# ljj7975/honk

Hardware: AMD Instinct MI355X
Metric: 1s-clips/sec (whole node) + top-1 acc, res15 12-label Speech Commands (higher is better)
Workload: dtype f16x2

## Files before the change

### honk_amd/csrc/res_bf16p.inc

```

#ifndef HONK_PAIR_PDM
#define HONK_PAIR_PDM 0
#endif
#ifndef HONK_PAIR_PKRELU
#define HONK_PAIR_PKRELU 1
#endif
#ifndef HONK_PAIR_MIX
#define HONK_PAIR_MIX 1
#endif

struct Block16PArgs {
  __bf16* R;
  const char* wA;
  const char* wB;
  unsigned chunk_bytes;
  int nclips, H, W;
  int d, lgd, sB;
  int lag;
  int NRA, NRB;
  int slotb;
  int ppr;
  float* chsum;
  int padb;
  int ringpad;
};

template <int NT, int SP>
struct G16P {
  static constexpr int P = 64;
  static constexpr int ZB = 256;
  static constexpr int PXB = 16 * ((G16W<NT, SP>::CB / 16 + 1) / 4 * 4 + 2);
};
static constexpr int g16p_pxb(int NT, int SP) { return 16 * ((32 * NT * SP / 16 + 1) / 4 * 4 + 2); }

static constexpr int g16p_lds_bytes() { return 160 * 1024; }
static constexpr int g16p_zb_tbl() { return 1024; }
static constexpr int g16p_tr() { return 32; }
static constexpr int g16p_teb() { return 32; }
static constexpr int g16p_lds_extra(bool tbl, int wps, int slotb) {
  return tbl ? g16p_zb_tbl() + 1024 + wps * g16p_tr() * g16p_teb() + slotb : 256 + 1024;
}
static constexpr int g16p_sink_off(int zb) { return ((zb > g16p_zb_tbl() ? zb : g16p_zb_tbl()) + 255) / 256 * 256; }
static constexpr int g16p_shared_bytes(int zb) { return g16p_sink_off(zb) + 1024; }
static constexpr int g16p_stream_bytes(int ns, int slotb) {
  return ((g16p_lds_bytes() - g16p_shared_bytes(slotb)) / ns) / 256 * 256;
}

template <int NT, int SP, int PPR, int PPW, int NS, bool LM, int FM, int SCA = 0, int SCB = 0, bool LIN = false>
__device__ __forceinline__ void block16p_body(const Block16PArgs& a) {
  using G = G16W<NT, SP, FM>;
  using Q = G16P<NT, SP>;
  constexpr int KSA = G::KSA, CB = G::CB, CP = G::CP, P = Q::P;
  constexpr int PD0 = ((FM == 2 || SCA > 0) && KSA % 7 == 0 && NS == 1) ? 6 : G::PD;
  constexpr int NOA = PD0 + 1;
  constexpr int PD = PD0 > 2 ? PD0 - HONK_PAIR_PDM : PD0;
  constexpr int PXB = Q::PXB;
  constexpr int MAXR = (2 * PPW + PPR - 1) / PPR;
  static_assert(KSA > PPW + 1, "DMA pieces ride on k-steps 1 .. PPW");
  __shared__ __attribute__((aligned(16))) char lds[g16p_lds_bytes()];

  const int tid = threadIdx.x;
  const int lane = tid & 63;
  const int wave = __builtin_amdgcn_readfirstlane(tid >> 6);
  constexpr int WPS = LM ? 2 : 4;
  const int stream = wave / WPS;
  const int role = LM ? 0 : ((wave >> 1) & 1) ^ ((HONK_PAIR_MIX && NS == 2) ? (stream & 1) : 0);
  const int widx = wave & 1;
  const int g = lane >> 4;
  const int i16 = lane & 15;

  const int GR = gridDim.x;
  const int bid = blockIdx.x;
  const int w0 = (int)(((long)bid * a.nclips) / GR);
  const int w1 = (int)(((long)(bid + 1) * a.nclips) / GR);
  if (w1 <= w0) return;
  const int per = (w1 - w0 + NS - 1) / NS;
  const int s0 = min(w0 + stream * per, w1);
  const int s1 = min(s0 + per, w1);
  int c0 = s0, c1 = s1;
  const int H = a.H, W = a.W, d = a.d, lgd = a.lgd;
  const int RB = W * CB;
  const unsigned clip_bytes = (unsigned)(H * RB);
  int rows_total = (c1 - c0) * H;
  int total = rows_total * W;
  const int qd = H >> lgd, rem = H & (d - 1);
  const int q1 = qd + 1;
  constexpr bool TBL = FM == 2 || (FM == 0 && SCA != 0);
  constexpr bool PADC = TBL && (LM || SCA > 0);
  const int padb = PADC ? a.padb : 0;
  constexpr int ZB = TBL ? g16p_zb_tbl() : Q::ZB;
  constexpr bool SHZ = NS > 1 && TBL && !LM;
  const int sbase = SHZ ? g16p_shared_bytes(a.slotb + a.ringpad) + stream * g16p_stream_bytes(NS, a.slotb + a.ringpad)
                        : stream * (g16p_lds_bytes() / NS);
  const int ringA = sbase, ringB = sbase + a.NRA * a.slotb;
  const int zoff = SHZ ? 0 : sbase + (a.NRA + a.NRB) * a.slotb + a.ringpad;
  const int dummy = SHZ ? g16p_sink_off(a.slotb + a.ringpad) : zoff + ZB;
  const int nsteps = ((LM ? 1 : per) * H * W + a.lag + P - 1) / P + 1;

  if ((wave & (WPS - 1)) == 0) {
    if constexpr (TBL) *(u32x4*)(lds + zoff + lane * 16) = u32x4{0u, 0u, 0u, 0u};
    else *(unsigned*)(lds + zoff + lane * 4) = 0u;
  }
  if constexpr (TBL) {
    const int zs = SHZ ? 0 : dummy + 1024 + WPS * g16p_tr() * g16p_teb();
    for (int o = ((wave & (WPS - 1)) * 64 + lane) * 16; o < a.slotb + a.ringpad; o += WPS * 1024)
      *(u32x4*)(lds + zs + o) = u32x4{0u, 0u, 0u, 0u};
    const int rings = PADC ? (a.NRA + a.NRB) * a.slotb + a.ringpad : 0;
    for (int o = ((wave & (WPS - 1)) * 64 + lane) * 16; o < rings; o += WPS * 1024)
      *(u32x4*)(lds + sbase + o) = u32x4{0u, 0u, 0u, 0u};
  }
  __builtin_amdgcn_s_waitcnt(0xc07f);
  __builtin_amdgcn_s_barrier();

  u32x4 wr[G::WP][KSA][NT];
  {
    const __amdgpu_buffer_rsrc_t wrs =
        __builtin_amdgcn_make_buffer_rsrc((void*)(role ? a.wB : a.wA), (short)0, G::WP * G::WPART, 0x00020000);
#pragma unroll
    for (int pt = 0; pt < G::WP; ++pt)
#pragma unroll
      for (int s = 0; s < KSA; ++s)
#pragma unroll
        for (int n = 0; n < NT; ++n) {
          const bool used = s < KSA - 1 || g < G::UGA;
          int voff = used ? lane * 16 : 0x40000000, soff = G::xfrag(pt, s, n);
          if (G::MERGE && s == KSA - 1 && pt == 0 && !used) {
            voff = (lane - 16 * G::UGA) * 16;
            soff = G::xfrag(1, s, n);
          }
          wr[pt][s][n] = __builtin_bit_cast(u32x4, __builtin_amdgcn_raw_buffer_load_b128(wrs, voff, soff, 0));
          if ((pt * KSA + s) * NT + n < (NS * WPS > 4 ? 32 : 64)) asm volatile("" : "+a"(wr[pt][s][n]));
        }
  }

  constexpr int CPT = 2 * NT;
  const int g16 = 16 * g;
  const int hi2 = g >= 2 ? -1 : 0;
  int lastc;
  {
    constexpr int S = KSA - 1, tA = (4 * S) / CPT;
    int cc[4];
#pragma unroll
    for (int gi = 0; gi < 4; ++gi) {
      const int gg = (G::MERGE && gi >= G::UGA) ? gi - G::UGA : gi;
      const int c = 4 * S + gg;
      cc[gi] = c < 18 * NT ? c - tA * CPT : 0;
    }
    const int ccg = g == 0 ? cc[0] : g == 1 ? cc[1] : g == 2 ? cc[2] : cc[3];
    lastc = 16 * ccg + 16 * CPT * tA - g16;
  }
  static_assert((4 * (KSA - 1) + 3) / CPT == (4 * (KSA - 1)) / CPT || 4 * (KSA - 1) + 3 >= 18 * NT,
                "the last k-step covers one tap");

  const int ring = role ? ringB : ringA;
  const int nr = role ? a.NRB : a.NRA;
  const int sr = role ? a.sB : 1;
  const int sc = role ? (a.sB << lgd) : d;
  const int scb = sc * PXB;

  struct Walk {
    int q, w, j, n, c;
    unsigned rowb;
    int sR, sO;
  };
  const unsigned dRB = (unsigned)(RB << lgd);
  const unsigned dclsd = (unsigned)RB - (unsigned)(qd - 1) * dRB, dcls1d = 0u - dRB;
  const unsigned dclip = clip_bytes - (unsigned)((d - 1) * RB) - (unsigned)(((d - 1) < rem ? q1 : qd) - 1) * dRB;
  const int ringRb = nr * a.slotb, ringOb = a.NRB * a.slotb, srb = sr * a.slotb;
  auto walk_init = [&](int q0) {
    Walk k;
    k.q = q0;
    const int qs = q0 >= 0 ? q0 : q0 + ((31 - q0) >> 5) * 32;
    const int r = qs / W;
    k.w = qs - r * W;
    const int cl = r / H;
    const int rl = r - cl * H;
    if (rl < rem * q1) {
      k.c = rl / q1;
      k.j = rl - k.c * q1;
      k.n = q1;
    } else {
      const int t = rl - rem * q1;
      const int cu = t / qd;
      k.c = rem + cu;
      k.j = t - cu * qd;
      k.n = qd;
    }
    k.rowb = (unsigned)(c0 + cl) * clip_bytes + (unsigned)((k.c + (k.j << lgd)) * RB);
    k.sR = (r % nr) * a.slotb;
    k.sO = (r % a.NRB) * a.slotb;
    return k;
  };
  auto row_adv = [&](Walk& k) {
    const int sR1 = k.sR + a.slotb, sO1 = k.sO + a.slotb;
    k.sR = sR1 == ringRb ? 0 : sR1;
    k.sO = sO1 == ringOb ? 0 : sO1;
    const int j1 = k.j + 1;
    const bool wj = j1 == k.n;
    const int c1 = k.c + (wj ? 1 : 0);
    const bool wc = c1 == d;
    unsigned inc = dRB;
    const unsigned dcls = dclsd + (k.n == q1 ? dcls1d : 0u);
    inc = wj ? dcls : inc;
    inc = wc ? dclip : inc;
    k.rowb += inc;
    k.j = wj ? 0 : j1;
    k.c = wc ? 0 : c1;
    k.n = k.c < rem ? q1 : qd;
  };
  constexpr bool WIDE = (PPR - 1) * 1024 >= 32 * PXB;
  auto walk_adv = [&](Walk& k) {
    if constexpr (WIDE) {
      const int w2 = k.w + (k.q >= 0 ? 32 : 0);
      const bool wrap = w2 >= W;
      k.w = wrap ? w2 - W : w2;
      const int sR1 = k.sR + (wrap ? a.slotb : 0), sO1 = k.sO + (wrap ? a.slotb : 0);
      k.sR = sR1 == ringRb ? 0 : sR1;
      k.sO = sO1 == ringOb ? 0 : sO1;
      const int j1 = k.j + (wrap ? 1 : 0);
      const bool wj = j1 == k.n;
      const int c1 = k.c + (wj ? 1 : 0);
      const bool wc = c1 == d;
      unsigned inc = wrap ? dRB : 0u;
      const unsigned dcls = dclsd + (k.n == q1 ? dcls1d : 0u);
      inc = wj ? dcls : inc;
      inc = wc ? dclip : inc;
      k.rowb += inc;
      k.j = wj ? 0 : j1;
      k.c = wc ? 0 : c1;
      k.n = k.c < rem ? q1 : qd;
    } else {
      if (k.q >= 0) {
        k.w += 32;
        while (k.w >= W) {
          k.w -= W;
          row_adv(k);
        }
      }
    }
    k.q += 32;
  };
  struct MG {
    int tq[9];
    unsigned pix;
    int lo;
  };
  auto geo = [&](const Walk& k) {
    MG m;
    const bool valid = k.q >= 0 && k.q < total;
    int sm = k.sR - srb, sp = k.sR + srb;
    sm = sm < 0 ? sm + ringRb : sm;
    sp = sp >= ringRb ? sp - ringRb : sp;
    const int wb = k.w * PXB + g16;
    const bool rok[3] = {valid && k.j >= sr, valid, valid && k.j + sr < k.n};
    const int rbase[3] = {ring + sm + wb, ring + k.sR + wb, ring + sp + wb};
    const bool cok[3] = {k.w >= sc, true, k.w + sc < W};
    const int zg = zoff + g16;
#pragma unroll
    for (int dy = 0; dy < 3; ++dy)
#pragma unroll
      for (int dx = 0; dx < 3; ++dx) {
        const int t = dy * 3 + dx;
        m.tq[t] = ((rok[dy] && cok[dx]) ? rbase[dy] + (dx - 1) * scb : zg) - 16 * CPT * t;
      }
    m.pix = valid ? k.rowb + (unsigned)(k.w * CB) : 0xF0000000u;
    m.lo = valid ? ringB + k.sO + k.w * PXB : dummy;
    return m;
  };

  constexpr int TR = g16p_tr(), TEB = g16p_teb();
  const int tbl = (SHZ ? sbase + (a.NRA + a.NRB) * a.slotb + a.ringpad : dummy + 1024) + (wave & (WPS - 1)) * (TR * TEB);
  const int zslot = SHZ ? 0 : dummy + 1024 + WPS * (TR * TEB);
  struct WalkT {
    int w, r;
    u32x4 e;
    int lo;
    int wb;
    bool okl, okr;
  };
  auto refill = [&](int tb) {
    const int r = tb + lane;
    int rb0 = zslot + padb, rb1 = zslot + padb, rb2 = zslot + padb, lo = -1;
    unsigned pix = 0xF0000000u;
    if (lane < TR && r >= 0 && r < rows_total) {
      const int cl = r / H, rl = r - cl * H;
      int c, j, n;
      if (rl < rem * q1) {
        c = rl / q1;
        j = rl - c * q1;
        n = q1;
      } else {
        const int t = rl - rem * q1, cu = t / qd;
        c = rem + cu;
        j = t - cu * qd;
        n = qd;
      }
      pix = (unsigned)(c0 + cl) * clip_bytes + (unsigned)((c + (j << lgd)) * RB);
      rb1 = ring + (r % nr) * a.slotb + padb;
      if (j >= sr) rb0 = ring + ((r - sr) % nr) * a.slotb + padb;
      if (j + sr < n) rb2 = ring + ((r + sr) % nr) * a.slotb + padb;
      lo = ringB + (r % a.NRB) * a.slotb + padb;
    }
    if (lane < TR) {
      char* e = lds + tbl + (r & (TR - 1)) * TEB;
      *(u32x4*)e = u32x4{(unsigned)rb0, (unsigned)rb1, (unsigned)rb2, pix};
      *(int*)(e + 16) = lo;
    }
  };
  auto floordiv = [](int x, int y) { return x >= 0 ? x / y : -((y - 1 - x) / y); };
  auto tread = [&](WalkT& k) {
    const char* e = lds + tbl + (k.r & (TR - 1)) * TEB;
    k.e = *(const u32x4*)e;
    k.lo = *(const int*)(e + 16);
    k.wb = __mul24(k.w, PXB) + g16;
    if constexpr (!PADC) {
      k.okl = k.w >= sc;
      k.okr = k.w + sc < W;
    }
  };
  auto walk_init_t = [&](int q0) {
    WalkT k;
    k.r = floordiv(q0, W);
    k.w = q0 - k.r * W;
    tread(k);
    return k;
  };
  constexpr int NWRAP = WIDE ? 1 : 3;
  auto walk_adv_t = [&](WalkT& k) {
    k.w += 32;
#pragma unroll
    for (int i = 0; i < NWRAP; ++i) {
      const bool wrap = k.w >= W;
      k.w = wrap ? k.w - W : k.w;
      k.r += wrap ? 1 : 0;
    }
    tread(k);
  };
  int tk[9];
#pragma unroll
  for (int t = 0; t < 9; ++t) tk[t] = (t % 3 - 1) * scb - 16 * CPT * t;
  const int zg0 = zoff + g16;
  auto scc_of = [](auto rolec) constexpr { return decltype(rolec)::value ? SCB : SCA; };
  auto biasc_of = [](auto rolec) constexpr {
    return (decltype(rolec)::value ? SCB : SCA) * PXB + 96;
  };
  auto geo_row = [&](auto rolec, const WalkT& k, MG& m, auto dyc) {
    constexpr int DY = decltype(dyc)::value;
    constexpr int SCC = scc_of(decltype(rolec){});
    const int rb = (int)k.e[DY] + k.wb;
    if constexpr (PADC && SCC > 0) {
      m.tq[DY] = rb - biasc_of(decltype(rolec){});
    } else if constexpr (PADC) {
#pragma unroll
      for (int dx = 0; dx < 3; ++dx) m.tq[DY * 3 + dx] = rb + tk[DY * 3 + dx];
    } else {
      const bool ok[3] = {k.okl, true, k.okr};
#pragma unroll
      for (int dx = 0; dx < 3; ++dx) m.tq[DY * 3 + dx] = ok[dx] ? rb + tk[DY * 3 + dx] : zg0;
    }
    if constexpr (DY == 2) {
      m.pix = k.e[3] + (unsigned)__mul24(k.w, CB);
      m.lo = k.lo >= 0 ? k.lo + k.wb - g16 : dummy;
    }
  };
  auto geo_t = [&](auto rolec, const WalkT& k) {
    MG m;
    static_for<3>([&](auto dyc) { geo_row(rolec, k, m, dyc); });
    return m;
  };
  auto lc_same = [&](auto rolec) { return hi2 & (scc_of(decltype(rolec){}) * PXB - 16 * CPT); };
  auto lc_next = [&](auto rolec) { return hi2 & (-2 * scc_of(decltype(rolec){}) * PXB - 16 * CPT); };
  auto aoff = [&](auto rolec, const int (&tq)[9], auto stc) {
    constexpr int S = decltype(stc)::value;
    constexpr int tA = (4 * S) / CPT;
    constexpr int SCC = scc_of(decltype(rolec){});
    if constexpr (PADC && SCC > 0) {
      if constexpr (S == KSA - 1) {
        return tq[tA / 3] + lastc - 16 * CPT * tA;
      } else {
        constexpr int tB = (4 * S + 3) / CPT;
        if constexpr (tA == tB) {
          return tq[tA / 3];
        } else if constexpr (tA / 3 == tB / 3) {
          return tq[tA / 3] + lc_same(rolec);
        } else {
          return ((tq[tB / 3] & hi2) | (tq[tA / 3] & ~hi2)) + lc_next(rolec);
        }
      }
    } else if constexpr (S == KSA - 1) {
      return tq[tA] + lastc - 64 * S;
    } else {
      constexpr int tB = (4 * S + 3) / CPT;
      if constexpr (tA == tB) {
        return tq[tA];
      } else {
        constexpr int GS = CPT * tB - 4 * S;
        static_assert(GS == 2, "NT = 3: every mixed k-step splits its lane groups 2 + 2");
        return (tq[tB] & hi2) | (tq[tA] & ~hi2);
      }
    }
  };

  auto imm_of = [](auto rolec, auto stc) constexpr {
    constexpr int S = decltype(stc)::value;
    constexpr int tA = (4 * S) / CPT;
    constexpr int SCC = decltype(rolec)::value ? SCB : SCA;
    constexpr int B = SCC * PXB + 96;
    if constexpr (S == KSA - 1) return B + (tA % 3 - 1) * SCC * PXB;
    else return B + (tA % 3 - 1) * SCC * PXB - 16 * CPT * tA + 64 * S;
  };

  u32x4 oa[NOA][SP];
  auto load_a = [&](auto rolec, const int (&tq)[9], auto stc, u32x4 (&o)[SP]) {
    constexpr int S = decltype(stc)::value;
    const int off = aoff(rolec, tq, stc);
    if constexpr (PADC && scc_of(decltype(rolec){}) > 0) {
      constexpr int IMM = imm_of(decltype(rolec){}, stc);
      static_assert(IMM >= 0 && IMM < 65536, "IMM: ds_read offset range");
#pragma unroll
      for (int pt = 0; pt < SP; ++pt) o[pt] = *(const u32x4*)(lds + off + IMM + pt * CP * 2);
    } else {
#pragma unroll
      for (int pt = 0; pt < SP; ++pt) o[pt] = *(const u32x4*)(lds + off + 64 * S + pt * CP * 2);
    }
  };

  f32x4 accs[2][NT];
  uint4 rvs[2][G::NRF][SP];
  unsigned ppix = 0xF0000000u;
  int plo = dummy;
#pragma unroll
  for (int q = 0; q < 2; ++q) {
#pragma unroll
    for (int n = 0; n < NT; ++n) accs[q][n] = f32x4{0.f, 0.f, 0.f, 0.f};
#pragma unroll
    for (int f = 0; f < G::NRF; ++f)
#pragma unroll
      for (int pt = 0; pt < SP; ++pt) rvs[q][f][pt] = uint4{0u, 0u, 0u, 0u};
  }
  const __amdgpu_buffer_rsrc_t rrs = __builtin_amdgcn_make_buffer_rsrc((void*)a.R, (short)0, a.chunk_bytes, 0x00020000);

  constexpr int NSTO = LM ? 0 : G::NS;
  constexpr int ELAST = LM ? NT - 1 : G::store_step(NSTO - 1);
  f32x4 csum[NT];
#pragma unroll
  for (int n = 0; n < NT; ++n) csum[n] = f32x4{0.f, 0.f, 0.f, 0.f};
  constexpr int KE = (KSA - ELAST - 2 >= 2) ? KSA - ELAST - 2 : 2;
  constexpr int KW = 4;
  constexpr int KG = KSA - 1 - PD - 1;
  static_assert(KG > KW && KG + PD < KSA, "walk schedule");
  constexpr bool BAL = false;
  constexpr int NHS = 2 * ELAST + 2;
  constexpr int KWT = PD > 2 ? 0 : 1, KET = PD > 2 ? 5 : 2, KGT = PD > 2 ? 2 : KET + NHS;
  static_assert(!(TBL && BAL) || (KGT + 2 + PD < KSA && KET + NHS <= KSA && KWT < KGT), "table walk schedule");

  typename ActT<FM>::V4 h[SP][NT];
  auto epi_store = [&](auto rolec, auto ic) {
    constexpr bool ISB = decltype(rolec)::value;
    constexpr int I = decltype(ic)::value;
    if constexpr (I < G::NPS) {
      constexpr int pr = I / SP, pt = I % SP;
      const u32x2 lo = __builtin_bit_cast(u32x2, h[pt][2 * pr]), hi = __builtin_bit_cast(u32x2, h[pt][2 * pr + 1]);
      const u32x4 v4{lo[0], lo[1], hi[0], hi[1]};
      if constexpr (ISB) {
        __builtin_amdgcn_raw_buffer_store_b128(v4, rrs, ppix + 16 * g, 64 * pr + pt * CP * 2, 0);
      } else {
        *(u32x4*)(lds + plo + 16 * g + 64 * pr + pt * CP * 2) = v4;
      }
    } else {
      constexpr int pt = I - G::NPS;
      const u32x2 v2 = __builtin_bit_cast(u32x2, h[pt][NT - 1]);
      if constexpr (ISB) {
        __builtin_amdgcn_raw_buffer_store_b64(v2, rrs, ppix + 8 * g, 64 * (NT / 2) + pt * CP * 2, 0);
      } else {
        *(u32x2*)(lds + plo + 8 * g + 64 * (NT / 2) + pt * CP * 2) = v2;
      }
    }
  };
  auto epi_step = [&](auto rolec, auto ec, auto pendc) {
    constexpr bool ISB = decltype(rolec)::value;
    constexpr int E = decltype(ec)::value;
    constexpr int PQ = decltype(pendc)::value;
    f32x4 (&accp)[NT] = accs[PQ];
    uint4 (&rv)[G::NRF][SP] = rvs[PQ];
    if constexpr (E < NT && !ISB && !LM && FM == 2 && HONK_PAIR_PKRELU) {
      constexpr int n = E;
      const f16x4 hv{(_Float16)accp[n][0], (_Float16)accp[n][1], (_Float16)accp[n][2], (_Float16)accp[n][3]};
      h[0][n] = __builtin_bit_cast(typename ActT<FM>::V4, __builtin_elementwise_maximum(hv, f16x4{0, 0, 0, 0}));
    } else if constexpr (E < NT) {
      constexpr int n = E;
      f32x4 v;
#pragma unroll
      for (int k = 0; k < 4; ++k) v[k] = relu_acc(accp[n][k]);
      if constexpr (ISB) {
        constexpr int f = n >> 1, e0 = (n < (NT & ~1)) ? (n & 1) * 4 : 0;
#pragma unroll
        for (int k = 0; k < 4; ++k) {
          const int e = e0 + k;
          if constexpr (SP == 1) {
            v[k] = add_res<FM>(v[k], rv[f][0][e >> 1], e);
          } else {
            const float r = act_dec<FM>(rv[f][0][e >> 1], e) + act_dec<FM>(rv[f][1][e >> 1], e);
            v[k] += r;
          }
        }
      }
      if constexpr (LM) {
        const bool ok = plo != dummy;
#pragma unroll
        for (int k = 0; k < 4; ++k) csum[n][k] += ok ? v[k] : 0.f;
      } else {
#pragma unroll
        for (int k = 0; k < 4; ++k) {
          h[0][n][k] = (typename ActT<FM>::T)v[k];
          if constexpr (SP == 2) h[SP - 1][n][k] = (__bf16)(v[k] - (float)h[0][n][k]);
        }
      }
    }
    static_for<NSTO>([&](auto ic) {
      if constexpr (G::store_step(decltype(ic)::value) == E) epi_store(rolec, ic);
    });
  };
  auto epi_half = [&](auto rolec, auto hc, auto pendc) {
    constexpr bool ISB = decltype(rolec)::value;
    constexpr int HS = decltype(hc)::value;
    constexpr int PQ = decltype(pendc)::value;
    if constexpr (HS < 2 * NT) {
      constexpr int n = HS / 2, k0 = 2 * (HS % 2);
      f32x4 (&accp)[NT] = accs[PQ];
      uint4 (&rv)[G::NRF][SP] = rvs[PQ];
#pragma unroll
      for (int k = k0; k < k0 + 2; ++k) {
        float v = relu_acc(accp[n][k]);
        if constexpr (ISB) {
          constexpr int f = n >> 1, e0 = (n < (NT & ~1)) ? (n & 1) * 4 : 0;
          const int e = e0 + k;
          if constexpr (SP == 1) {
            v = add_res<FM>(v, rv[f][0][e >> 1], e);
          } else {
            const float r = act_dec<FM>(rv[f][0][e >> 1], e) + act_dec<FM>(rv[f][1][e >> 1], e);
            v += r;
          }
        }
        if constexpr (LM) {
          csum[n][k] += plo != dummy ? v : 0.f;
        } else {
          h[0][n][k] = (typename ActT<FM>::T)v;
          if constexpr (SP == 2) h[SP - 1][n][k] = (__bf16)(v - (float)h[0][n][k]);
        }
      }
    }
    static_for<NSTO>([&](auto ic) {
      if constexpr (2 * G::store_step(decltype(ic)::value) + 1 == HS) epi_store(rolec, ic);
    });
  };

  auto res_loads = [&](uint4 (&rvn)[G::NRF][SP], unsigned po) {
#pragma unroll
    for (int f = 0; f < G::NRF; ++f)
#pragma unroll
      for (int pt = 0; pt < SP; ++pt) {
        if (f < NT / 2) {
          rvn[f][pt] =
              __builtin_bit_cast(uint4, __builtin_amdgcn_raw_buffer_load_b128(rrs, po + 16 * g, 64 * f + pt * CP * 2, 0));
        } else {
          const u32x2 t =
              __builtin_bit_cast(u32x2, __builtin_amdgcn_raw_buffer_load_b64(rrs, po + 8 * g, 64 * f + pt * CP * 2, 0));
          rvn[f][pt] = uint4{t[0], t[1], 0u, 0u};
        }
      }
  };

  struct RowCur {
    int cl, c, j, n, slot;
  };
  auto cur_adv = [&](RowCur& r) {
    r.slot = r.slot + 1 == a.NRA ? 0 : r.slot + 1;
    if (++r.j == r.n) {
      r.j = 0;
      if (++r.c == d) {
        r.c = 0;
        ++r.cl;
      }
      r.n = r.c < rem ? q1 : qd;
    }
  };
  auto cur_off = [&](const RowCur& r) {
    return (unsigned)(c0 + r.cl) * clip_bytes + (unsigned)((r.c + (r.j << lgd)) * RB);
  };
  unsigned psrc[(PPR + 1) / 2];
#pragma unroll
  for (int i = 0; i < (PPR + 1) / 2; ++i) psrc[i] = 0;
#pragma unroll
  for (int t = 0; t < PPR; ++t) {
    const int ch = 64 * t + lane, px = ch / (PXB / 16), wi = ch - px * (PXB / 16);
    const unsigned v = (px < W && wi < CB / 16) ? (unsigned)(px * CB + wi * 16) : 0xffffu;
    psrc[t >> 1] |= v << (16 * (t & 1));
  }
  auto dma = [&](unsigned off, int slot, auto pac, auto pbc, bool ok) {
    constexpr int PA = decltype(pac)::value, PB = decltype(pbc)::value;
    const int part = widx ? PB : PA;
    const unsigned va = (psrc[PA >> 1] >> (16 * (PA & 1))) & 0xffffu, vb = (psrc[PB >> 1] >> (16 * (PB & 1))) & 0xffffu;
    const unsigned v = widx ? vb : va;
    const int dst = ok ? ringA + slot + padb + part * 1024 : dummy;
    __builtin_amdgcn_raw_ptr_buffer_load_lds(rrs,
                                             (__attribute__((address_space(3))) void*)(lds + __builtin_amdgcn_readfirstlane(dst)),
                                             16, (v == 0xffffu || !ok) ? 0xF0000000u : off + v, 0, 0, 0);
  };
  const int PW = P / W, PR = P - PW * W;
  int frow = (P + 31) / W, fcol = (P + 31) - ((P + 31) / W) * W;
  auto frontier = [&]() { return frow + 1 < rows_total - 1 ? frow + 1 : rows_total - 1; };
  RowCur rc{0, 0, 0, rem > 0 ? q1 : qd, 0};
  auto restart = [&]() {
    rows_total = (c1 - c0) * H;
    total = rows_total * W;
    frow = (P + 31) / W;
    fcol = (P + 31) - ((P + 31) / W) * W;
    rc = RowCur{0, 0, 0, rem > 0 ? q1 : qd, 0};
    plo = dummy;
    ppix = 0xF0000000u;
  };
  unsigned roff[MAXR];
  int rslot[MAXR];
  static_assert(!LIN || (!LM && TBL && !PADC), "LIN: the two-stream row-table pair");
  const unsigned lsb0 = (unsigned)c0 * clip_bytes;
  const int lnpr = LIN ? a.NRA * a.slotb / 1024 : 1;
  const int lptot = LIN ? (rows_total * RB + 1023) / 1024 : 0;
  int lpdone = 0, lpb = 0;
  unsigned lsrc = 0;
  auto lin_need = [&](int f) {
    const int p = ((f + 1) * RB + 1023) / 1024;
    return p < lptot ? p : lptot;
  };
  auto lin_dma = [&](int j, int nnew) {
    const bool ok = j < nnew;
    int rp = lpb + j;
    rp = rp >= lnpr ? rp - lnpr : rp;
    const int dst = ok ? ringA + rp * 1024 : dummy;
    __builtin_amdgcn_raw_ptr_buffer_load_lds(
        rrs, (__attribute__((address_space(3))) void*)(lds + __builtin_amdgcn_readfirstlane(dst)), 16,
        ok ? lsrc + (unsigned)j * 1024u + (unsigned)lane * 16u : 0xF0000000u, 0, 0, 0);
  };
  constexpr bool DMAB = false;

  constexpr int DSP = 1;
  auto dma_piece = [](int S) constexpr {
    return (S >= 1 && (S - 1) % DSP == 0 && (S - 1) / DSP < PPW) ? (S - 1) / DSP : -1;
  };
  static_assert(1 + DSP * (PPW - 1) < KSA, "DMA pieces inside the first m-tile");
  auto vm_after_dma = []() constexpr {
    int n = G::NRL + NSTO;
    for (int i = 0; i < NSTO; ++i) {
      int ks = (TBL && BAL) ? KET + 2 * G::store_step(i) + 1 : KE + G::store_step(i);
      if (ks > KSA - 1) ks = KSA - 1;
      if (ks >= 1 + DSP * (PPW - 1)) ++n;
    }
    return n;
  };
  auto run_mtile = [&](auto rolec, auto parc, const MG& cur, MG& nxt, auto& wk, int nnew) {
    constexpr bool ISB = decltype(rolec)::value;
    constexpr int PAR = decltype(parc)::value;
    constexpr bool FIRST = PAR == 0;
    f32x4 (&acc)[NT] = accs[PAR];
    static_for<KSA>([&](auto stc) {
      constexpr int S = decltype(stc)::value;
      constexpr int SN = S + PD;
      if constexpr (SN < KSA) load_a(rolec, cur.tq, KStep<SN>{}, oa[SN % NOA]);
      else load_a(rolec, nxt.tq, KStep<SN - KSA>{}, oa[SN % NOA]);
      __builtin_amdgcn_sched_barrier(0);
      if constexpr (ISB && S == 0) res_loads(rvs[PAR], cur.pix);
      if constexpr (TBL && BAL) {
        if constexpr (S == KWT) walk_adv_t(wk);
        if constexpr (S >= KGT && S < KGT + 3) geo_row(rolec, wk, nxt, std::integral_constant<int, S - KGT>{});
      } else if constexpr (TBL) {
        if constexpr (S == KW) walk_adv_t(wk);
        if constexpr (S == KG) nxt = geo_t(rolec, wk);
      } else {
        if constexpr (S == KW) walk_adv(wk);
        if constexpr (S == KG) nxt = geo(wk);
      }
      const u32x4 (&ac)[SP] = oa[S % NOA];
      constexpr int NPROD = S == KSA - 1 ? G::NPROD_LAST : G::PRODUCTS;
      static_for<NPROD>([&](auto tc) {
        constexpr int T = decltype(tc)::value;
        constexpr int WP = G::wpart(T), XP = G::xpart(T);
        static_for<NT>([&](auto nc) {
          constexpr int N = decltype(nc)::value;
          mfma_w<S == 0 && T == 0, FM == 2>(acc[N], wr[WP][S][N], ac[XP]);
        });
      });
      if constexpr (LIN && !ISB && FIRST && dma_piece(S) >= 0) {
        lin_dma(2 * dma_piece(S) + widx, nnew);
      } else if constexpr (ISB == DMAB && FIRST && dma_piece(S) >= 0) {
        constexpr int i = dma_piece(S);
        constexpr int ra = (2 * i) / PPR, rb = (2 * i + 1) / PPR;
        constexpr int pa = (2 * i) % PPR, pb = (2 * i + 1) % PPR;
        const int rr = widx ? rb : ra;
        dma(widx ? roff[rb] : roff[ra], widx ? rslot[rb] : rslot[ra], std::integral_constant<int, pa>{},
            std::integral_constant<int, pb>{}, rr < nnew);
      }
      if constexpr (TBL && BAL) {
        if constexpr (S >= KET && S < KET + NHS)
          epi_half(rolec, std::integral_constant<int, S - KET>{}, std::integral_constant<int, 1 - PAR>{});
      } else {
        static_for<ELAST + 1>([&](auto ec) {
          constexpr int E = decltype(ec)::value;
          if constexpr ((KE + E < KSA ? KE + E : KSA - 1) == S) epi_step(rolec, ec, std::integral_constant<int, 1 - PAR>{});
        });
      }
      static_for<NPROD * NT>([&](auto) {
        __builtin_amdgcn_sched_group_barrier(0x008, 1, 0);
        __builtin_amdgcn_sched_group_barrier(0x002, 2, 0);
        __builtin_amdgcn_sched_group_barrier(0x004, 2, 0);
      });
      __builtin_amdgcn_sched_barrier(0);
    });
  };

  auto run_role = [&](auto rolec) {
    constexpr bool ISB = decltype(rolec)::value;
    int fprev = frontier();
    if constexpr (LIN && !ISB) {
      lpdone = lin_need(fprev);
      for (int p = widx; p < lpdone; p += 2)
        __builtin_amdgcn_raw_ptr_buffer_load_lds(
            rrs, (__attribute__((address_space(3))) void*)(lds + __builtin_amdgcn_readfirstlane(ringA + p * 1024)), 16,
            lsb0 + (unsigned)p * 1024u + (unsigned)lane * 16u, 0, 0, 0);
    } else if constexpr (!ISB) {
      for (int row = 0; row <= fprev; ++row) {
        if ((row & 1) == widx) {
          const unsigned ro = cur_off(rc);
          const int so = ringA + rc.slot * a.slotb + padb;
#pragma unroll
          for (int t = 0; t < PPR; ++t) {
            const unsigned v = (psrc[t >> 1] >> (16 * (t & 1))) & 0xffffu;
            __builtin_amdgcn_raw_ptr_buffer_load_lds(
                rrs, (__attribute__((address_space(3))) void*)(lds + __builtin_amdgcn_readfirstlane(so + t * 1024)), 16,
                v == 0xffffu ? 0xF0000000u : ro + v, 0, 0, 0);
          }
        }
        cur_adv(rc);
      }
    } else if constexpr (DMAB) {
      for (int row = 0; row <= fprev; ++row) cur_adv(rc);
    }
    const int q0w = (ISB ? -a.lag - P : 0) + 16 * widx;
    int qlim = 0;
    if constexpr (TBL) {
      const int tb = floordiv(q0w, W);
      refill(tb);
      qlim = (tb + TR) * W;
    }
    auto wk = [&]() {
      if constexpr (TBL) return walk_init_t(q0w + i16);
      else return walk_init(q0w + i16);
    }();
    MG mgs[2];
    if constexpr (TBL) mgs[0] = geo_t(rolec, wk);
    else mgs[0] = geo(wk);
    for (int k = 0; k < nsteps; ++k) {
      asm volatile("" ::: "memory");
      if constexpr (!ISB) wait_vmcnt<0>();
      else if constexpr (DMAB) wait_vmcnt<vm_after_dma()>();
      __builtin_amdgcn_s_waitcnt(0xc07f);
      __builtin_amdgcn_s_barrier();
      asm volatile("" ::: "memory");
      if constexpr (TBL) {
        const int qs = q0w + k * P;
        if (qs + P + 15 >= qlim) {
          const int tb = floordiv(qs, W);
          refill(tb);
          qlim = (tb + TR) * W;
        }
      }
      if (k == 0) static_for<PD>([&](auto stc) { load_a(rolec, mgs[0].tq, stc, oa[decltype(stc)::value]); });
      int nnew = 0;
      if constexpr (LIN && !ISB) {
        fcol += PR;
        frow += PW;
        if (fcol >= W) {
          fcol -= W;
          ++frow;
        }
        const int need = lin_need(frontier());
        nnew = need - lpdone;
        lpb = lpdone % lnpr;
        lsrc = lsb0 + (unsigned)lpdone * 1024u;
        lpdone = need;
      } else if constexpr (ISB == DMAB) {
        fcol += PR;
        frow += PW;
        if (fcol >= W) {
          fcol -= W;
          ++frow;
        }
        const int fcur = frontier();
        nnew = fcur - fprev;
        RowCur t = rc;
#pragma unroll
        for (int m = 0; m < MAXR; ++m) {
          roff[m] = cur_off(t);
          rslot[m] = t.slot * a.slotb;
          if (m + 1 < MAXR) cur_adv(t);
        }
        for (int m = 0; m < nnew; ++m) cur_adv(rc);
        fprev = fcur;
      }
      static_for<2>([&](auto itc) {
        constexpr int IT = decltype(itc)::value;
        run_mtile(rolec, std::integral_constant<int, IT>{}, mgs[IT], mgs[1 - IT], wk, nnew);
        ppix = mgs[IT].pix;
        plo = mgs[IT].lo;
      });
    }
    wait_vmcnt<0>();
    static_for<ELAST + 1>([&](auto ec) { epi_step(rolec, ec, std::integral_constant<int, 1>{}); });
  };

  if constexpr (LM) {
    for (int ci = 0; ci < per; ++ci) {
      c0 = s0 + ci;
      c1 = c0 < s1 ? c0 + 1 : c0;
      restart();
      asm volatile("" ::: "memory");
      __builtin_amdgcn_s_waitcnt(0xc07f);
      __builtin_amdgcn_s_barrier();
      asm volatile("" ::: "memory");
      run_role(std::integral_constant<bool, false>{});
      float* cs = a.chsum + ((size_t)(c0 < c1 ? c0 : 0) * 2 + widx) * CP;
#pragma unroll
      for (int n = 0; n < NT; ++n) {
        f32x4 c;
#pragma unroll
        for (int k = 0; k < 4; ++k) {
          c[k] = sum16_dpp(csum[n][k]);
        }
        if (c0 < c1 && i16 == 0) *(f32x4*)(cs + co16(NT, n, 4 * g)) = c;
        csum[n] = f32x4{0.f, 0.f, 0.f, 0.f};
      }
    }
  } else {
    if (role == 0) run_role(std::integral_constant<bool, false>{});
    else run_role(std::integral_constant<bool, true>{});
  }
}

template <int NT, int SP, int PPR, int PPW, int NS, int FM = (SP == 2 ? 1 : 0), int SCA = 0, int SCB = 0,
          bool LIN = false>
__global__ __launch_bounds__(256 * NS, 1) void block16p_kernel(Block16PArgs a) {
  block16p_body<NT, SP, PPR, PPW, NS, false, FM, SCA, SCB, LIN>(a);
}

template <int NT, int SP, int PPR, int PPW, int NS, int FM = (SP == 2 ? 1 : 0), int SCL = 0>
__global__ __launch_bounds__(128 * NS, 1) void block16l_kernel(Block16PArgs a) {
  block16p_body<NT, SP, PPR, PPW, NS, true, FM, SCL, SCL>(a);
}
```

### honk_amd/csrc/res_vf.hip

```cpp
#define HONK_RES_VF_TU 1
#include "res.hip"

namespace honk {
namespace res {

bool launch_pair_vf(int FM, int ppr, bool imm, int dA, int dB, dim3 gd, dim3 bd, hipStream_t st,
                    const Block16PArgs& pa) {
  if ((FM == 2 || FM == 0) && imm) {
#define HONK_PI(a_, b_)                                                                              \
  if (dA == a_ && dB == b_) {                                                                        \
    if (FM == 2) hipLaunchKernelGGL((block16p_kernel<3, 1, 4, 4, 1, 2, a_, b_>), gd, bd, 0, st, pa); \
    else hipLaunchKernelGGL((block16p_kernel<3, 1, 4, 4, 1, 0, a_, b_>), gd, bd, 0, st, pa);        \
    return true;                                                                                     \
  }
    HONK_PI(1, 1) HONK_PI(1, 2) HONK_PI(2, 2) HONK_PI(4, 4) HONK_PI(4, 8) HONK_PI(8, 8)
#undef HONK_PI
    return false;
  }
  if (FM == 1 && ppr == 9) hipLaunchKernelGGL((block16p_kernel<3, 2, 9, 9, 1>), gd, bd, 0, st, pa);
  else if (FM == 1 && ppr == 5) hipLaunchKernelGGL((block16p_kernel<3, 2, 5, 10, 1>), gd, bd, 0, st, pa);
  else if (FM == 1) hipLaunchKernelGGL((block16p_kernel<3, 2, 3, 9, 1>), gd, bd, 0, st, pa);
  else if (FM == 2 && ppr == 4) hipLaunchKernelGGL((block16p_kernel<3, 1, 4, 4, 1, 2>), gd, bd, 0, st, pa);
  else if (FM == 2) hipLaunchKernelGGL((block16p_kernel<3, 1, 2, 5, 1, 2>), gd, bd, 0, st, pa);
  else if (ppr == 4) hipLaunchKernelGGL((block16p_kernel<3, 1, 4, 4, 1>), gd, bd, 0, st, pa);
  else hipLaunchKernelGGL((block16p_kernel<3, 1, 2, 5, 1>), gd, bd, 0, st, pa);
  return true;
}

void launch_pair2t_vf(int ppr, bool lin, dim3 gd, dim3 bd, hipStream_t st, const Block16PArgs& pa) {
  if (lin) hipLaunchKernelGGL((block16p_kernel<3, 1, 2, 4, 2, 0, -1, -1, true>), gd, bd, 0, st, pa);
  else if (ppr == 4) hipLaunchKernelGGL((block16p_kernel<3, 1, 4, 4, 2, 0, -1, -1>), gd, bd, 0, st, pa);
  else hipLaunchKernelGGL((block16p_kernel<3, 1, 2, 5, 2, 0, -1, -1>), gd, bd, 0, st, pa);
}

bool launch_pair2i_vf(int dA, int dB, dim3 gd, dim3 bd, hipStream_t st, const Block16PArgs& pa) {
#define HONK_P2I(a_, b_)                                                              \
  if (dA == a_ && dB == b_) {                                                         \
    hipLaunchKernelGGL((block16p_kernel<3, 1, 4, 4, 2, 0, a_, b_>), gd, bd, 0, st, pa); \
    return true;                                                                      \
  }
  HONK_P2I(1, 1) HONK_P2I(1, 2) HONK_P2I(2, 2) HONK_P2I(4, 4) HONK_P2I(8, 8)
#undef HONK_P2I
  return false;
}

bool launch_pairk_vf(int dA, int dB, dim3 gd, dim3 bd, hipStream_t st, const Block16PArgs& pa) {
#define HONK_PK(a_, b_)                                                       \
  if (dA == a_ && dB == b_) {                                                 \
    hipLaunchKernelGGL((block16k_kernel<a_, b_>), gd, bd, 0, st, pa);        \
    return true;                                                              \
  }
  HONK_PK(1, 1) HONK_PK(1, 2) HONK_PK(2, 2) HONK_PK(4, 4) HONK_PK(4, 8) HONK_PK(8, 8)
#undef HONK_PK
  return false;
}

void launch_last_vf(int FM, int d, dim3 gd, dim3 bd, hipStream_t st, const Block16PArgs& pa) {
  if (FM == 1) hipLaunchKernelGGL((block16l_kernel<3, 2, 9, 9, 2>), gd, bd, 0, st, pa);
  else if (FM == 2 && d == 16) hipLaunchKernelGGL((block16l_kernel<3, 1, 4, 4, 2, 2, 16>), gd, bd, 0, st, pa);
  else if (FM == 0 && d == 16 && pa.padb > 0) hipLaunchKernelGGL((block16l_kernel<3, 1, 4, 4, 2, 0, 16>), gd, bd, 0, st, pa);
  else if (FM == 2) hipLaunchKernelGGL((block16l_kernel<3, 1, 4, 4, 2, 2>), gd, bd, 0, st, pa);
  else hipLaunchKernelGGL((block16l_kernel<3, 1, 4, 4, 2>), gd, bd, 0, st, pa);
}

}
}
```

Before: 315,000.

## Precompute DMA row descriptors inside previous m-tile and narrow A-role table reads

```diff
diff --git a/honk_amd/csrc/res_bf16p.inc b/honk_amd/csrc/res_bf16p.inc
--- a/honk_amd/csrc/res_bf16p.inc
+++ b/honk_amd/csrc/res_bf16p.inc
@@ -7,6 +7,9 @@
 #endif
 #ifndef HONK_PAIR_MIX
 #define HONK_PAIR_MIX 1
+#endif
+#ifndef HONK_PAIR_DTOP
+#define HONK_PAIR_DTOP 0
 #endif
 
 struct Block16PArgs {
@@ -308,9 +311,15 @@
     }
   };
   auto floordiv = [](int x, int y) { return x >= 0 ? x / y : -((y - 1 - x) / y); };
-  auto tread = [&](WalkT& k) {
+  typedef unsigned u32x3 __attribute__((ext_vector_type(3)));
+  auto tread = [&](auto rolec, WalkT& k) {
     const char* e = lds + tbl + (k.r & (TR - 1)) * TEB;
-    k.e = *(const u32x4*)e;
+    if constexpr (decltype(rolec)::value) {
+      k.e = *(const u32x4*)e;
+    } else {
+      const u32x3 e3 = *(const u32x3*)e;
+      k.e = u32x4{e3[0], e3[1], e3[2], 0xF0000000u};
+    }
     k.lo = *(const int*)(e + 16);
     k.wb = __mul24(k.w, PXB) + g16;
     if constexpr (!PADC) {
@@ -318,15 +327,15 @@
       k.okr = k.w + sc < W;
     }
   };
-  auto walk_init_t = [&](int q0) {
+  auto walk_init_t = [&](auto rolec, int q0) {
     WalkT k;
     k.r = floordiv(q0, W);
     k.w = q0 - k.r * W;
-    tread(k);
+    tread(rolec, k);
     return k;
   };
   constexpr int NWRAP = WIDE ? 1 : 3;
-  auto walk_adv_t = [&](WalkT& k) {
+  auto walk_adv_t = [&](auto rolec, WalkT& k) {
     k.w += 32;
 #pragma unroll
     for (int i = 0; i < NWRAP; ++i) {
@@ -334,7 +343,7 @@
       k.w = wrap ? k.w - W : k.w;
       k.r += wrap ? 1 : 0;
     }
-    tread(k);
+    tread(rolec, k);
   };
   int tk[9];
 #pragma unroll
@@ -572,21 +581,26 @@
   };
 
   struct RowCur {
-    int cl, c, j, n, slot;
-  };
-  auto cur_adv = [&](RowCur& r) {
-    r.slot = r.slot + 1 == a.NRA ? 0 : r.slot + 1;
-    if (++r.j == r.n) {
-      r.j = 0;
-      if (++r.c == d) {
-        r.c = 0;
-        ++r.cl;
-      }
-      r.n = r.c < rem ? q1 : qd;
-    }
-  };
-  auto cur_off = [&](const RowCur& r) {
-    return (unsigned)(c0 + r.cl) * clip_bytes + (unsigned)((r.c + (r.j << lgd)) * RB);
+    int c, j, n;
+    unsigned off;
+    int slot;
+  };
+  const int ringAb = a.NRA * a.slotb;
+  auto cur_adv = [&](RowCur& r, int by) {
+    const int s1 = r.slot + (by ? a.slotb : 0);
+    r.slot = s1 == ringAb ? 0 : s1;
+    const int j1 = r.j + by;
+    const bool wj = j1 == r.n;
+    const int c1 = r.c + (wj ? 1 : 0);
+    const bool wc = c1 == d;
+    unsigned inc = by ? dRB : 0u;
+    const unsigned dcls = dclsd + (r.n == q1 ? dcls1d : 0u);
+    inc = wj ? dcls : inc;
+    inc = wc ? dclip : inc;
+    r.off += inc;
+    r.j = wj ? 0 : j1;
+    r.c = wc ? 0 : c1;
+    r.n = r.c < rem ? q1 : qd;
   };
   unsigned psrc[(PPR + 1) / 2];
 #pragma unroll
@@ -610,18 +624,35 @@
   const int PW = P / W, PR = P - PW * W;
   int frow = (P + 31) / W, fcol = (P + 31) - ((P + 31) / W) * W;
   auto frontier = [&]() { return frow + 1 < rows_total - 1 ? frow + 1 : rows_total - 1; };
-  RowCur rc{0, 0, 0, rem > 0 ? q1 : qd, 0};
+  RowCur rc{0, 0, rem > 0 ? q1 : qd, (unsigned)c0 * clip_bytes, 0};
   auto restart = [&]() {
     rows_total = (c1 - c0) * H;
     total = rows_total * W;
     frow = (P + 31) / W;
     fcol = (P + 31) - ((P + 31) / W) * W;
-    rc = RowCur{0, 0, 0, rem > 0 ? q1 : qd, 0};
+    rc = RowCur{0, 0, rem > 0 ? q1 : qd, (unsigned)c0 * clip_bytes, 0};
     plo = dummy;
     ppix = 0xF0000000u;
   };
+  int fprev = 0, nnew = 0;
   unsigned roff[MAXR];
   int rslot[MAXR];
+  static_assert(MAXR + 2 < KSA, "desc_row(m) rides on k-step 2 + m");
+  auto desc_front = [&]() {
+    fcol += PR;
+    frow += PW;
+    const bool wrap = fcol >= W;
+    fcol -= wrap ? W : 0;
+    frow += wrap ? 1 : 0;
+    const int fcur = frontier();
+    nnew = fcur - fprev;
+    fprev = fcur;
+  };
+  auto desc_row = [&](int m) {
+    roff[m] = rc.off;
+    rslot[m] = rc.slot;
+    cur_adv(rc, m < nnew ? 1 : 0);
+  };
   static_assert(!LIN || (!LM && TBL && !PADC), "LIN: the two-stream row-table pair");
   const unsigned lsb0 = (unsigned)c0 * clip_bytes;
   const int lnpr = LIN ? a.NRA * a.slotb / 1024 : 1;
@@ -632,6 +663,19 @@
     const int p = ((f + 1) * RB + 1023) / 1024;
     return p < lptot ? p : lptot;
   };
+  auto lin_next = [&]() {
+    fcol += PR;
+    frow += PW;
+    const bool wrap = fcol >= W;
+    fcol -= wrap ? W : 0;
+    frow += wrap ? 1 : 0;
+    const int need = lin_need(frontier());
+    lpb += nnew;
+    lpb -= lpb >= lnpr ? lnpr : 0;
+    lsrc += (unsigned)nnew * 1024u;
+    nnew = need - lpdone;
+    lpdone = need;
+  };
   auto lin_dma = [&](int j, int nnew) {
     const bool ok = j < nnew;
     int rp = lpb + j;
@@ -641,22 +685,14 @@
         rrs, (__attribute__((address_space(3))) void*)(lds + __builtin_amdgcn_readfirstlane(dst)), 16,
         ok ? lsrc + (unsigned)j * 1024u + (unsigned)lane * 16u : 0xF0000000u, 0, 0, 0);
   };
-  constexpr bool DMAB = false;
 
   constexpr int DSP = 1;
   auto dma_piece = [](int S) constexpr {
     return (S >= 1 && (S - 1) % DSP == 0 && (S - 1) / DSP < PPW) ? (S - 1) / DSP : -1;
   };
   static_assert(1 + DSP * (PPW - 1) < KSA, "DMA pieces inside the first m-tile");
-  auto vm_after_dma = []() constexpr {
-    int n = G::NRL + NSTO;
-    for (int i = 0; i < NSTO; ++i) {
-      int ks = (TBL && BAL) ? KET + 2 * G::store_step(i) + 1 : KE + G::store_step(i);
-      if (ks > KSA - 1) ks = KSA - 1;
-      if (ks >= 1 + DSP * (PPW - 1)) ++n;
-    }
-    return n;
-  };
+  constexpr int VM_AFTER_RES = NSTO + G::NRL;
+  static_assert(G::store_step(0) >= 1 || NSTO == 0, "no store ahead of the first residual use");
   auto run_mtile = [&](auto rolec, auto parc, const MG& cur, MG& nxt, auto& wk, int nnew) {
     constexpr bool ISB = decltype(rolec)::value;
     constexpr int PAR = decltype(parc)::value;
@@ -667,13 +703,14 @@
       constexpr int SN = S + PD;
       if constexpr (SN < KSA) load_a(rolec, cur.tq, KStep<SN>{}, oa[SN % NOA]);
       else load_a(rolec, nxt.tq, KStep<SN - KSA>{}, oa[SN % NOA]);
-      __builtin_amdgcn_sched_barrier(0);
+      constexpr bool DTOP = HONK_PAIR_DTOP && !ISB && FIRST;
+      if constexpr (!(DTOP && S <= 1)) __builtin_amdgcn_sched_barrier(0);
       if constexpr (ISB && S == 0) res_loads(rvs[PAR], cur.pix);
       if constexpr (TBL && BAL) {
-        if constexpr (S == KWT) walk_adv_t(wk);
+        if constexpr (S == KWT) walk_adv_t(rolec, wk);
         if constexpr (S >= KGT && S < KGT + 3) geo_row(rolec, wk, nxt, std::integral_constant<int, S - KGT>{});
       } else if constexpr (TBL) {
-        if constexpr (S == KW) walk_adv_t(wk);
+        if constexpr (S == KW) walk_adv_t(rolec, wk);
         if constexpr (S == KG) nxt = geo_t(rolec, wk);
       } else {
         if constexpr (S == KW) walk_adv(wk);
@@ -691,7 +728,7 @@
       });
       if constexpr (LIN && !ISB && FIRST && dma_piece(S) >= 0) {
         lin_dma(2 * dma_piece(S) + widx, nnew);
-      } else if constexpr (ISB == DMAB && FIRST && dma_piece(S) >= 0) {
+      } else if constexpr (!ISB && FIRST && dma_piece(S) >= 0) {
         constexpr int i = dma_piece(S);
         constexpr int ra = (2 * i) / PPR, rb = (2 * i + 1) / PPR;
         constexpr int pa = (2 * i) % PPR, pb = (2 * i + 1) % PPR;
@@ -699,38 +736,56 @@
         dma(widx ? roff[rb] : roff[ra], widx ? rslot[rb] : rslot[ra], std::integral_constant<int, pa>{},
             std::integral_constant<int, pb>{}, rr < nnew);
       }
+      if constexpr (!ISB && !FIRST) {
+        if constexpr (LIN) {
+          if constexpr (S == 1) lin_next();
+        } else {
+          if constexpr (S == 1) desc_front();
+          if constexpr (S >= 2 && S < 2 + MAXR) desc_row(S - 2);
+        }
+      }
       if constexpr (TBL && BAL) {
         if constexpr (S >= KET && S < KET + NHS)
           epi_half(rolec, std::integral_constant<int, S - KET>{}, std::integral_constant<int, 1 - PAR>{});
       } else {
         static_for<ELAST + 1>([&](auto ec) {
           constexpr int E = decltype(ec)::value;
-          if constexpr ((KE + E < KSA ? KE + E : KSA - 1) == S) epi_step(rolec, ec, std::integral_constant<int, 1 - PAR>{});
+          if constexpr ((KE + E < KSA ? KE + E : KSA - 1) == S) {
+            if constexpr (ISB && E == 0) wait_vmcnt<VM_AFTER_RES>();
+            epi_step(rolec, ec, std::integral_constant<int, 1 - PAR>{});
+          }
         });
       }
+      if constexpr (DTOP && S <= 1) __builtin_amdgcn_sched_group_barrier(0x100, 1, 0);
       static_for<NPROD * NT>([&](auto) {
         __builtin_amdgcn_sched_group_barrier(0x008, 1, 0);
         __builtin_amdgcn_sched_group_barrier(0x002, 2, 0);
-        __builtin_amdgcn_sched_group_barrier(0x004, 2, 0);
+        __builtin_amdgcn_sched_group_barrier(0x004, (DTOP && S <= 1) ? 5 : 2, 0);
       });
-      __builtin_amdgcn_sched_barrier(0);
+      if constexpr (!(DTOP && S == 0)) __builtin_amdgcn_sched_barrier(0);
     });
   };
 
   auto run_role = [&](auto rolec) {
     constexpr bool ISB = decltype(rolec)::value;
-    int fprev = frontier();
+    if constexpr (!ISB) {
+      fprev = frontier();
+      nnew = 0;
+    }
     if constexpr (LIN && !ISB) {
       lpdone = lin_need(fprev);
       for (int p = widx; p < lpdone; p += 2)
         __builtin_amdgcn_raw_ptr_buffer_load_lds(
             rrs, (__attribute__((address_space(3))) void*)(lds + __builtin_amdgcn_readfirstlane(ringA + p * 1024)), 16,
             lsb0 + (unsigned)p * 1024u + (unsigned)lane * 16u, 0, 0, 0);
+      lpb = lpdone % lnpr;
+      lsrc = lsb0 + (unsigned)lpdone * 1024u;
+      lin_next();
     } else if constexpr (!ISB) {
       for (int row = 0; row <= fprev; ++row) {
         if ((row & 1) == widx) {
-          const unsigned ro = cur_off(rc);
-          const int so = ringA + rc.slot * a.slotb + padb;
+          const unsigned ro = rc.off;
+          const int so = ringA + rc.slot + padb;
 #pragma unroll
           for (int t = 0; t < PPR; ++t) {
             const unsigned v = (psrc[t >> 1] >> (16 * (t & 1))) & 0xffffu;
@@ -739,10 +794,11 @@
                 v == 0xffffu ? 0xF0000000u : ro + v, 0, 0, 0);
           }
         }
-        cur_adv(rc);
-      }
-    } else if constexpr (DMAB) {
-      for (int row = 0; row <= fprev; ++row) cur_adv(rc);
+        cur_adv(rc, 1);
+      }
+      desc_front();
+#pragma unroll
+      for (int m = 0; m < MAXR; ++m) desc_row(m);
     }
     const int q0w = (ISB ? -a.lag - P : 0) + 16 * widx;
     int qlim = 0;
@@ -752,16 +808,16 @@
       qlim = (tb + TR) * W;
     }
     auto wk = [&]() {
-      if constexpr (TBL) return walk_init_t(q0w + i16);
+      if constexpr (TBL) return walk_init_t(rolec, q0w + i16);
       else return walk_init(q0w + i16);
     }();
     MG mgs[2];
     if constexpr (TBL) mgs[0] = geo_t(rolec, wk);
     else mgs[0] = geo(wk);
+    if constexpr (ISB) wait_vmcnt<0>();
     for (int k = 0; k < nsteps; ++k) {
       asm volatile("" ::: "memory");
       if constexpr (!ISB) wait_vmcnt<0>();
-      else if constexpr (DMAB) wait_vmcnt<vm_after_dma()>();
       __builtin_amdgcn_s_waitcnt(0xc07f);
       __builtin_amdgcn_s_barrier();
       asm volatile("" ::: "memory");
@@ -774,38 +830,6 @@
         }
       }
       if (k == 0) static_for<PD>([&](auto stc) { load_a(rolec, mgs[0].tq, stc, oa[decltype(stc)::value]); });
-      int nnew = 0;
-      if constexpr (LIN && !ISB) {
-        fcol += PR;
-        frow += PW;
-        if (fcol >= W) {
-          fcol -= W;
-          ++frow;
-        }
-        const int need = lin_need(frontier());
-        nnew = need - lpdone;
-        lpb = lpdone % lnpr;
-        lsrc = lsb0 + (unsigned)lpdone * 1024u;
-        lpdone = need;
-      } else if constexpr (ISB == DMAB) {
-        fcol += PR;
-        frow += PW;
-        if (fcol >= W) {
-          fcol -= W;
-          ++frow;
-        }
-        const int fcur = frontier();
-        nnew = fcur - fprev;
-        RowCur t = rc;
-#pragma unroll
-        for (int m = 0; m < MAXR; ++m) {
-          roff[m] = cur_off(t);
-          rslot[m] = t.slot * a.slotb;
-          if (m + 1 < MAXR) cur_adv(t);
-        }
-        for (int m = 0; m < nnew; ++m) cur_adv(rc);
-        fprev = fcur;
-      }
       static_for<2>([&](auto itc) {
         constexpr int IT = decltype(itc)::value;
         run_mtile(rolec, std::integral_constant<int, IT>{}, mgs[IT], mgs[1 - IT], wk, nnew);
diff --git a/honk_amd/csrc/res_vf.hip b/honk_amd/csrc/res_vf.hip
--- a/honk_amd/csrc/res_vf.hip
+++ b/honk_amd/csrc/res_vf.hip
@@ -1,4 +1,7 @@
 #define HONK_RES_VF_TU 1
+#ifndef HONK_PAIR_DTOP
+#define HONK_PAIR_DTOP 1
+#endif
 #include "res.hip"
 
 namespace honk {
```

Measured after the change: 328,000 (median of 6 runs). 1.04x the previous value.
